# m-hamza-mughal/RAG-Gesture

Measured on AMD Instinct MI355X. Metric: SMPL-X frames/sec, len150 DDIM-50 + insertion guidance; 1/2/4/8 GPU, higher is better.
Workload: dtype bf16

## Files before the change

include/rg_gesture.h:

```cpp
#ifndef RG_GESTURE_H
#define RG_GESTURE_H

#include <stdint.h>

#ifdef __cplusplus
extern "C" {
#endif

typedef struct rg_handle rg_handle;

enum rg_status {
  RG_OK = 0,
  RG_ERR_INVALID = -1,
  RG_ERR_HIP = -2,
  RG_ERR_NO_DEVICE = -3
};

#define RG_VERSION 123
int rg_version(void);
int rg_create(rg_handle** out, int device);
void rg_destroy(rg_handle* h);
const char* rg_last_error(rg_handle* h);
int rg_num_cus(rg_handle* h);

int rg_ddim_update(rg_handle* h, const float* x, const float* x0, float* x_out, int64_t n,
                   float c_recip, float c_recipm1, float c_a, float c_b, void* stream);

int rg_cfg_ddim_update(rg_handle* h, const float* out, const float* x, float* x_out, float* x0_out,
                       const float* js, int B, int T, int D, float w_c, float w_u,
                       float c_recip, float c_recipm1, float c_a, float c_b, void* stream);
int rg_cfg_ddim_update_rows(rg_handle* h, const float* out_cond, const float* out_uncond, const float* x, float* x_out,
                            float* x_out2, const float* js, int B, int T, int D, float w_c, float w_u,
                            float c_recip, float c_recipm1, float c_a, float c_b, void* stream);

int rg_cfg_ddpm_update(rg_handle* h, const float* out, const float* x, const float* noise, float* x_out,
                       const float* js, int B, int T, int D, float w_c, float w_u, float c1, float c2, float sigma,
                       void* stream);

typedef struct rg_glue_args {
  const float* out_c_a;
  const float* out_u_a;
// ... 156 lines not shown
  const void* ustream;
  const void* afrag;
  const float* x;
  const float* tbias;
  const float* src_mask;
  const float* qmask;
  float* head;
  float* dump;
  float* xbuf;
  void* gbuf;
  const int* form;
  int L, B, T, S;
  int step, step_b, split;
  int dump_stage, dump_layer;
  int pairs;
  int twin;
  int* glue_ctr;
  rg_glue_args glue;
} rg_seq_args;

int rg_seq_forward(rg_handle* h, const rg_seq_args* args_host, void* stream);
int rg_seq2_forward(rg_handle* h, const rg_seq_args* args_host, void* stream);

#define RG_LANE_STRIDE 32
int rg_seqx_forward(rg_handle* h, const rg_seq_args* args_host, void* stream);
int rg_lane_form(rg_handle* h, int* state, int lane, int nlanes, int narrow_wgs, int wide_wgs, int budget, void* stream);

typedef struct rg_venc_args {
  const void* wstream;
  const void* pstream;
  const float* x;
  float* out;
  float* xbuf;
  float* dump;
  int nseq, S, nb, dump_block;
  const int* post_rows;
  float* post_mu;
  float* post_logvar;
  int post_nrows, pad_;
} rg_venc_args;

int rg_venc_forward(rg_handle* h, const rg_venc_args* args_host, void* stream);
int rg_venc_forward_grouped(rg_handle* h, const rg_venc_args* args_host, int n, void* stream);

typedef struct rg_vdec_args {
  const void* wstream;
// ... 429 lines not shown
```

rag-gesture_amd/csrc/rg_seq.hip:

```cpp
#ifndef RG_SEQ_BODY_ONLY
#define RG_PACK2_ONE
#endif
#include "rg_common.h"
#include "rg_stationary.h"
#include "rg_tail.h"
#include "rg_seq_host.h"

namespace {

constexpr int RD = 7;
constexpr int UPL = RG_SEQ_UPL;
constexpr int OFF_P0 = 0;
constexpr int OFF_P1 = TP * 1024;
constexpr int OFF_RING = 2 * TP * 1024;
constexpr int MAX_SEG = 8 * 34 + 5;
constexpr int OFF_DESC = OFF_RING + NW * RD * 1024;
constexpr int OFF_STAT = OFF_DESC + MAX_SEG * 16;
constexpr int LDS_BYTES = OFF_STAT + NW * TP * 2 * 4;
static_assert(LDS_BYTES <= 160 * 1024, "LDS budget");

#define U(name) U_##name = RG_SEQ_U_##name
enum { U(KV), U(KV2), U(Q), U(SAO), U(MIXX), U(Q3_0), U(MIX_0), U(Q3_1), U(MIX_1), U(Q3_2), U(MIX_2), U(FF1_0), U(FF2_0), U(FF1_1), U(FF2_1), U(FFO) };
#undef U
#define SEG(u, k) ((u) << 2 | (k))
// ... 460 lines not shown
  Acc out;
  zero(out);
  unit(out, P0, TL);
#pragma unroll
  for (int tb = 0; tb < 3; ++tb) {
    const int t = 16 * tb + l15;
    if (t < T) {
#pragma unroll
      for (int j = 0; j < 4; ++j) {
        const size_t o = ((size_t)seq * T + t) * DM + 64 * wave + 16 * j + 4 * g4;
        rg_tail::store_head(a.head, (unsigned)(o * 4), out[j][tb]);
      }
    }
  }
  wait_vmcnt<0>();
#ifdef RG_STAMPS
  if (a.dump_stage == 99 && lane0 == 0) {
    tacc[5] = __builtin_amdgcn_s_memrealtime() - tk0;
    for (int i = 0; i < 6; ++i) a.dump[(seq * 8 + wave) * 8 + i] = (float)tacc[i];
  }
#endif
}

__device__ __forceinline__ void seq_block(const rg_seq_args& a, const int block, const int pairs, unsigned char* const smem) {
  const int B = a.B;
  int seq0 = block;
  if (!pairs && (B & 3) == 0) {
    const int x = block & 7, q = block >> 3;
    seq0 = x < 4 ? 4 * q + x : B + 4 * q + (x - 4);
  }
  const int npass = pairs ? 2 : 1;
#pragma unroll 1
  for (int pass = 0; pass < npass; ++pass) {
    run_sequence(a, seq0 + pass * B, smem);
    __syncthreads();
    int* const ctr = rg_tail::late_ctr();
    if (ctr && !a.dump_stage) {
      const int c = seq0 + pass * B - (seq0 + pass * B >= B ? B : 0);
      rg_tail::arrive_and_glue<NTH>(ctr, c, c, reinterpret_cast<int*>(smem), __builtin_amdgcn_readfirstlane(threadIdx.x >> 6));
    }
  }
}

#ifndef RG_SEQ_BODY_ONLY
__global__ void __launch_bounds__(NTH) rg_seq_kernel(const rg_seq_args a) {
  extern __shared__ __attribute__((aligned(16))) unsigned char smem[];
  RG_OWN_THE_SIMD();
  seq_block(a, blockIdx.x, a.pairs, smem);
}

extern "C" int rg_seq_forward(rg_handle* h, const rg_seq_args* args_host, void* stream) {
  const std::string why = rg_seq_refusal(RG_SEQ_ENTRY, args_host);
  if (!why.empty()) { if (h) h->err = why; return RG_ERR_INVALID; }
  const rg_seq_args& a = *args_host;
  static rg_attr_once lds_once;
  RG_RESERVE_LDS(h, lds_once, rg_seq_kernel, LDS_BYTES);
  rg_prof_scope prof(h, stream, 3, rg_seq_flops(a));
  hipLaunchKernelGGL(rg_seq_kernel, dim3(a.pairs ? a.B : 2 * a.B), dim3(NTH), LDS_BYTES, rg_stream(stream), a);
  RG_CHECK_LAUNCH(h);
  prof.stop();
  return RG_OK;
}
#endif
```

rag-gesture_amd/csrc/rg_seq_host.h:

```cpp
#pragma once
#include <string>

#include "../../include/rg_gesture.h"

struct rg_seq_entry { const char *name, *need_bufs, *need_form, *no_dump, *twin_range, *twin_pairs, *no_twin; };
constexpr rg_seq_entry RG_SEQ_ENTRY = {"rg_seq_forward", nullptr, nullptr, nullptr, nullptr, nullptr, nullptr};
constexpr rg_seq_entry RG_SEQ2_ENTRY = {"rg_seq2_forward", "the two-sequence forward needs its scratch buffers xbuf and gbuf", nullptr,
                                        nullptr, "twin must be 0 or 1", "twin and pairs are two launch forms: set one of them", nullptr};
constexpr rg_seq_entry RG_SEQX_ENTRY = {
    "rg_seqx_forward", "the two-sequence form needs its scratch buffers xbuf and gbuf", "form: the lane's flag (rg_lane_form) must be given",
    "diagnostic dumps: use rg_seq_forward / rg_seq2_forward", nullptr, nullptr,
    "the twin form (one clip per workgroup) is not one of the device-chosen forms: use rg_seq2_forward"};

inline bool rg_seq_glue_ok(const rg_seq_args& a) {
  if (!a.glue_ctr) return true;
  const rg_glue_args& g = a.glue;
  if (a.dump_stage || g.n_a < 0 || g.n_b < 0 || g.n_a + g.n_b != a.B || g.T != a.T || g.D != 512 || !g.js || g.g_iter_next < 0) return false;
  if (g.n_a && !(g.out_c_a && g.out_u_a && g.x_a)) return false;
  if (g.n_b && !(g.out_c_b && g.out_u_b && g.x_b)) return false;
  return !g.in_seq_next || g.noise_next;
}

inline std::string rg_seq_refusal(const rg_seq_entry& e, const rg_seq_args* args) {
  const char* why = nullptr;
  if (!args) {
    why = "null args";
  } else {
    const rg_seq_args& a = *args;
    if (!(a.wstream && a.pstream && a.ustream && a.afrag && a.x && a.tbias && a.src_mask && a.qmask && a.head)) why = "null pointer";
    else if (e.need_bufs && !(a.xbuf && a.gbuf)) why = e.need_bufs;
    else if (e.need_form && !a.form) why = e.need_form;
    else if (!(a.L >= 1 && a.L <= 8 && a.B >= 1 && a.T >= 1 && a.T <= 48)) why = "unsupported shape (T <= 48, L <= 8)";
    else if (!(a.step >= 0 && a.step < a.S && a.step_b >= 0 && a.step_b < a.S)) why = "step out of range";
    else if (e.no_dump && a.dump_stage != 0) why = e.no_dump;
    else if (!e.no_dump && a.dump_stage != 0 && !a.dump) why = "dump_stage needs a dump buffer";
    else if (!(a.pairs == 0 || a.pairs == 1)) why = "pairs must be 0 or 1";
    else if (e.twin_range && !(a.twin == 0 || a.twin == 1)) why = e.twin_range;
    else if (e.twin_pairs && a.twin && a.pairs) why = e.twin_pairs;
    else if (e.no_twin && a.twin) why = e.no_twin;
    else if (!rg_seq_glue_ok(a)) why = "glue_ctr: glue must cover the B clips (n_a + n_b == B, T, D = 512), its pointers set, no dump";
  }
  return why ? std::string(e.name) + ": " + why : std::string();
}

inline double rg_seq_flops(const rg_seq_args& a) {
  const double unit = 2.0 * a.T * 512 * 512, att = 2.0 * a.T * 32 * 32 * 16;
  const double cond = (RG_SEQ_UPL * a.L + 2) * unit + a.L * (2 + 3) * att, unc = (10 * a.L + 2) * unit + a.L * 2 * att;
  return a.B * (cond + unc);
}
```

rag-gesture_amd/csrc/rg_tail.h:

```cpp
#pragma once
#include "rg_common.h"
#include <cstddef>

namespace rg_tail {

typedef __attribute__((ext_vector_type(4))) float f32x4;
typedef __attribute__((ext_vector_type(4))) unsigned u32x4;
constexpr int COHERENT = 17;

__device__ __forceinline__ float ddim_one(float x, float x0, float c_recip, float c_recipm1, float c_a, float c_b) {
#pragma clang fp contract(off)
  float eps = (c_recip * x - x0) / c_recipm1;
  return x0 * c_a + c_b * eps;
}
__device__ __forceinline__ float cfg_one(float oc, float ou, float jc, float ju, float w_c, float w_u) {
#pragma clang fp contract(off)
  return oc * w_c * jc + ou * w_u * ju;
}

template <typename P>
__device__ __forceinline__ P* uniform_ptr(P* p) {
  const unsigned long long v = reinterpret_cast<unsigned long long>(p);
  return reinterpret_cast<P*>((unsigned long long)__builtin_amdgcn_readfirstlane((unsigned)(v >> 32)) << 32 |
                              (unsigned)__builtin_amdgcn_readfirstlane((unsigned)v));
// ... 119 lines not shown
          const float4 v = glue_elem(a, k, C[i][h], U[i][h], X[i][h], jc[i], ju, ins, Y[i][h], E[i][h], two_over_numel);
          gstore(x0 + o, lane + 64 * h, v);
          if (x2_0) gstore(x2_0 + o, lane + 64 * h, v);
        }
      }
    }
  }
}

__device__ __forceinline__ float two_over_numel(const rg_glue_args& a) {
#pragma clang fp contract(off)
  const int rows_a = a.n_a * a.T;
  return 2.0f / ((float)rows_a * (float)a.D);
}

template <typename T>
__device__ __forceinline__ T late_arg(const unsigned offset) {
  auto p = (const __attribute__((address_space(4))) char*)__builtin_amdgcn_kernarg_segment_ptr();
  asm volatile("" : "+s"(p));
  T v;
  __builtin_memcpy(&v, p + offset, sizeof(T));
  return v;
}
__device__ __forceinline__ int* late_ctr() { return late_arg<int*>(offsetof(rg_seq_args, glue_ctr)); }

__device__ __forceinline__ void store_head(float* head, const unsigned byte_offset, const f32x4 v) {
  const auto rs = __builtin_amdgcn_make_buffer_rsrc(head, 0, 0x7fffffff, 0x00020000);
  __builtin_amdgcn_raw_buffer_store_b128(__builtin_bit_cast(u32x4, v), rs, byte_offset, 0, COHERENT);
}

template <int NTH>
__device__ __forceinline__ void arrive_and_glue(int* const ctr, const int c0, const int c1, int* const flag, const int wave) {
  const int lane = __builtin_amdgcn_mbcnt_hi(~0u, __builtin_amdgcn_mbcnt_lo(~0u, 0u));
  if (wave == 0 && lane == 0) {
    int m = 0;
    if (__hip_atomic_fetch_add(ctr + c0, 1, __ATOMIC_RELAXED, __HIP_MEMORY_SCOPE_AGENT) & 1) m |= 1;
    if (c1 != c0 && (__hip_atomic_fetch_add(ctr + c1, 1, __ATOMIC_RELAXED, __HIP_MEMORY_SCOPE_AGENT) & 1)) m |= 2;
    *flag = m;
  }
  __syncthreads();
  const int m = *flag;
  __syncthreads();
  if (m == 0) return;
  const rg_glue_args g = late_arg<rg_glue_args>(offsetof(rg_seq_args, glue));
  const float ton = two_over_numel(g);
#pragma unroll 1
  for (int q = 0; q < 2; ++q) {
    if (!(m >> q & 1)) continue;
    const int c = q ? c1 : c0;
    const bool ga = c < g.n_a;
    const int cl = ga ? c : c - g.n_a;
    glue_clip<NTH / 64>(g, ga, cl, wave, lane, ton);
  }
}

template <int NTH>
__device__ __forceinline__ void glue_own(const int c, const int wave) {
  const int lane = __builtin_amdgcn_mbcnt_hi(~0u, __builtin_amdgcn_mbcnt_lo(~0u, 0u));
  const rg_glue_args g = late_arg<rg_glue_args>(offsetof(rg_seq_args, glue));
  const bool ga = c < g.n_a;
  glue_clip<NTH / 64>(g, ga, ga ? c : c - g.n_a, wave, lane, two_over_numel(g));
}
}
```

rag-gesture_amd/denoiser.py:

```python
import math

import numpy as np
import torch

from . import capi, gemm as G, seqfwd as SQ

CONDS = ("xf_text", "xf_audio", "xf_spk")
BLOCKS = ("sa_block", "ca_blocks.xf_text", "ca_blocks.xf_audio", "ca_blocks.xf_spk", "ffn")


def _timestep_embedding(timesteps, dim, max_period=10000):
    half = dim // 2
    freqs = torch.exp(-math.log(max_period) * torch.arange(0, half, dtype=torch.float32) / half)
    args = timesteps[:, None].float() * freqs[None]
    return torch.cat([torch.cos(args), torch.sin(args)], dim=-1)


class DenoiserWeights:

    KV_GROUP = 2

    @staticmethod
    def _fold_ln(W, b, gamma, beta, pw, f32):
        Wp = (W.double() * gamma.double()[None, :]).float()
# ... 319 lines not shown
            pool[key] = torch.empty(*shape, device=self.w.dev, dtype=dtype)
        return pool[key]

    def chain_end(self):
        if self.sq is not None:
            self.sq.chain_end()

    def forward(self, x, step, step_b=None, split=None, glue=None):
        w, h, B, R, M, D, T = self.w, self.h, self.B, self.R, self.M, self.w.D, self.w.T
        if split is not None and not (0 < split < B):
            step, step_b, split = (step if split >= B else step_b), None, None
        if self.sq is not None:
            if glue is not None and not x.is_contiguous():
                raise capi.RgError("DenoiserSession.forward(glue=...): x is updated in place and must be contiguous")
            return self.sq.run(x.contiguous(), step, step_b, split, glue=glue)
        if glue is not None:
            raise capi.RgError("DenoiserSession.forward(glue=...): the sequence-stationary engine only")
        if self.ln_mode == "auto":
            out = self._forward_guarded(x, step)
            if split is None:
                return out
        return self._forward_chain(x, step, step_b, split)

    LN_GUARD_SIGMAS = 3.0

    def _forward_guarded(self, x, step):
        if torch.cuda.is_current_stream_capturing():
            raise capi.RgError("DenoiserSession(ln_mode='auto'): run one forward before capturing a graph")
        self._guard = torch.zeros(1, device=self.w.dev)
        self.ln_mode = "folded"
        out = self._forward_chain(x, step)
        self.ln_ratio = float(self._guard.item())
        self._guard = None
        if self.ln_ratio > self.LN_GUARD_SIGMAS ** 2:
            self.ln_mode, self.xa_bf = "prologue", None
            out = self._forward_chain(x, step)
        return out

    def _guard_stats(self, stats):
        if getattr(self, "_guard", None) is not None:
            self.h.call("ln_guard", stats, self.M, stats.shape[1], self.w.D, self._guard)

    def _forward_chain(self, x, step, step_b=None, split=None):
        w, h, B, R, M, D, T = self.w, self.h, self.B, self.R, self.M, self.w.D, self.w.T
        two = split is not None
        if two and (self.abf is None or self.hcat is None):
# ... 114 lines not shown
```

rag-gesture_amd/pipeline.py:

```python
import collections
import ctypes
import contextlib
import copy
import os
import time
import types

import torch
import yaml

from . import capi, denoiser, sampler, schedule as sched_mod, seqfwd, vae as vae_mod

MODELS = {}


def register_module(cls):
    MODELS[cls.__name__] = cls
    return cls


def register_with_mmcv(force=False):
    regs = []
    try:
        from mmcv.cnn import MODELS as mmcv_models
# ... 253 lines not shown
        self._ready()
        return {k: copy.deepcopy(v, memo) for k, v in dict.items(self) if k not in self._PLAIN}

    def __reduce__(self):
        self._ready()
        return (dict, (), None, None, iter([(k, v) for k, v in dict.items(self) if k not in self._PLAIN]))


@register_module
class MotionDiffusion(torch.nn.Module):

    profile_phases = False
    rotation_lanes = None
    form_lanes = None
    _cur_rot = None
    _last_state = None

    def __init__(self, model=None, loss_recon=None, loss_gen=None, loss_contact=None, loss_laplace=None,
                 diffusion_train=None, diffusion_test=None, init_cfg=None, inference_type="ddpm",
                 genloss_acceleration_weight=True, genloss_hands_weight=2, genloss_smooth=True,
                 body_part_lossweights=None, device="cuda", precision="bf16", lanes=2, sample_lanes=None, session_options=None,
                 vae_options=None, async_results=False, slots=2, max_inflight=2, cobatch_lanes="batch", base_lanes=8,
                 batch_lanes=4, lane_streams=None, calibrate_lanes=True, decode_stream=False, dynamic_forms=False, dynamic_budget=None, invert_alone_wide=True, tail_glue=True,
                 cache_exemplar_latents=True, exemplar_cache_bytes=8 << 30, skip_clip_encode=True, grouped_decode=True, **kwargs):
        super().__init__()
        self.grouped_decode = bool(grouped_decode)
        self.cache_exemplar_latents, self.exemplar_cache_bytes = bool(cache_exemplar_latents), int(exemplar_cache_bytes)
        self.skip_clip_encode = bool(skip_clip_encode)
        self.model = build_submodule(model, device=device, **kwargs)
        dt = dict(diffusion_test)
        self.schedule = sched_mod.Schedule(beta_scheduler=dt["beta_scheduler"], diffusion_steps=dt["diffusion_steps"],
                                           respace=dt.get("respace"))
        capi.require(dt.get("model_mean_type", "start_x") == "start_x" and dt.get("classifier_free_guidance_scale", 0) == 0,
                "unsupported argument: requires dt.get(\"model_mean_type\", \"start_x\") == \"start_x\" and dt.get(\"classifier_free_guidance_scale\", 0) == 0")
        self.inference_type = inference_type
        capi.require(inference_type in ("ddim", "ddpm"), "inference_type is 'ddim' (shipped config) or 'ddpm'")
        self.device, self.precision = torch.device(device), precision
        self.training = False
        self.session_options, self.vae_options = dict(session_options or {}), dict(vae_options or {})
        self.vae_options.setdefault("grouped_decode", self.grouped_decode)
        self._state = None
        self._sessions = {}
        self._graphs = {}
        self.use_graphs = True
        self.graph_captures = self.graph_cross_stream_waits = 0
        self._jitter = None
        self.phase_ms = {}
        self.lanes = int(lanes)
# ... 61 lines not shown

    def state_dict(self, *args, destination=None, prefix="", keep_vars=False):
        out = collections.OrderedDict() if destination is None else destination
        for k, v in (self._state or {}).items():
            out[prefix + "model." + k] = v
        return out

    _RECORD = True

    @staticmethod
    def _used_on(stream, *tensors):
        if not MotionDiffusion._RECORD:
            return
        for t in tensors:
            if torch.is_tensor(t) and t.is_cuda:
                t.record_stream(stream)

    def _graph_run(self, key, inputs, fn, owner=None):
        cur = torch.cuda.current_stream()
        self._used_on(cur, *inputs.values())
        if not self.use_graphs:
            return fn(inputs)
        if owner is not None:
            key = key + self._form_tag(self._session_opts(owner[0], owner[1], owner[2]))
        ent = self._graphs.pop(key, None)
        if ent is not None:
            self._graphs[key] = ent
        if ent is None:
            torch.cuda.synchronize()
            while len(self._graphs) >= self.MAX_GRAPHS:
                old = next(iter(self._graphs))
                del self._graphs[old]
                self._graph_owner.pop(old, None)
            if owner is not None:
                self._graph_owner[key] = owner
            static = {k: (None if v is None else torch.empty(v.shape, dtype=v.dtype, device=v.device).copy_(v))
                      for k, v in inputs.items()}
            side = torch.cuda.Stream()
            side.wait_stream(cur)
            with torch.cuda.stream(side):
                fn(static)
            cur.wait_stream(side)
            for k, v in inputs.items():
                if v is not None:
                    static[k].copy_(v)
            graph = torch.cuda.CUDAGraph()
            with capi.capture(graph):
# ... 39 lines not shown
        yield
        torch.cuda.synchronize()
        self.phase_ms[name] = self.phase_ms.get(name, 0.0) + (time.perf_counter() - t0) * 1e3

    def cuda(self, *a, **k):
        return self

    def cpu(self):
        return self

    def to(self, *a, **k):
        return self

    MAX_SESSIONS, MAX_GRAPHS = 192, 768

    def _session(self, B, role="sample", lane=0):
        opts = self._session_opts(B, role, lane)
        key = (B, role, lane, self._slot) + self._form_tag(opts)
        if key not in self._sessions:
            while len(self._sessions) >= self.MAX_SESSIONS:
                old = next(iter(self._sessions))
                torch.cuda.synchronize()
                del self._sessions[old]
                for gk in [g for g, o in self._graph_owner.items() if o == old[:4]]:
                    self._graphs.pop(gk, None)
                    del self._graph_owner[gk]
            self._sessions[key] = denoiser.DenoiserSession(self.model.weights, B, **opts)
        else:
            self._sessions[key] = self._sessions.pop(key)
        return self._sessions[key]

    LANE_SLOTS = 32

    @staticmethod
    def _form_tag(opts):
        return (bool(opts.get("seq_pairs")), opts.get("seq_duo"), "lane_dyn" in opts, bool(opts.get("seq_twin")))

    def _session_opts(self, B, role, lane):
        opts = dict(self.session_options)
        opts.setdefault("tail_glue", self.tail_glue)
        may_twin, twin = bool(opts.get("seq_twin", True)), False
        if opts.get("seq_pairs", "auto") == "auto":
            opts["seq_pairs"], duo = self._seq_form_auto(B)
            twin = may_twin and not opts["seq_pairs"] and bool(duo) and opts.get("seq_duo") is None
            if opts.get("seq_duo") is None:
                opts["seq_duo"] = duo
            if opts["seq_pairs"] and opts["seq_duo"] and role == "invert":
# ... 253 lines not shown
            prev_latent = prev_latent.to(dev).float()
            masked = torch.zeros_like(prev_latent)
            for idx in (up_i, ha_i, fa_i, lt_i):
                h.call("copy_rows", prev_latent, masked, B, 1, D, T, idx[-1], T, idx[0])
            prev_latent = masked

        ddpm = self.inference_type == "ddpm"
        in_seq = None
        if use_prev_latent and prev_latent is not None and not ddpm:
            in_seq = prev_latent
        elif use_outpaint and not ddpm:
            in_seq = retrieval_motion_latents
        x, start_noise, invl, inseq_noise, ddpm_noise = draw_batch_noise(
            tape, dev, B, T, D, S, use_inversion, use_insertion_guidance, visualize_inversion, ddpm, in_seq is not None,
            [len(retrieval_dict["retr_uncropped_latents"][b]) for b in range(B)] if use_inversion and visualize_inversion else ())
        st = types.SimpleNamespace(
            B=B, T=T, D=D, S=S, n_lat=n_lat, plan=plan, plan_s=plan_s, main=main, run_async=run_async, results=results,
            retrieval_dict=retrieval_dict, x=x, start_noise=start_noise, invl=invl, in_seq=in_seq, inseq_noise=inseq_noise,
            ddpm=ddpm, ddpm_noise=ddpm_noise, x_out=torch.empty(B, T, D, device=dev), use_inversion=use_inversion,
            use_insertion_guidance=use_insertion_guidance, guidance_iters=guidance_iters, guidance_lr=guidance_lr,
            visualize_inversion=visualize_inversion, inversion_start_time=inversion_start_time, vis_inv=[], vis_pairs=[],
            word=word, audio=audio, spk=spk, motion_mask=motion_mask, qmask=qmask, early_cond=early_cond,
            use_prev_latent=use_prev_latent, prev_latent=prev_latent, idx_groups=(up_i, ha_i, fa_i, lt_i), slot=self._slot, pid=pid, seq=self._submitted, via_submit=cob is not None,
            prev_future=prev_future if in_seq is not None else None, latent_ready=None)
        st.handle = self._last_state = types.SimpleNamespace(B=B, x_out=st.x_out, latent_ready=None)
        if cob is not None:
            st.word, st.audio, st.spk = (t.to(dev).clone() for t in (word, audio, spk))
            return self._submit_chain(st)
        self._inversion_pass(st)
        self._sampling_pass(st)
        return self._tail(st)

    def pending_latent(self):
        if self._last_state is None:
            raise capi.RgError("pending_latent(): no batch has been submitted")
        return PendingLatent(self._last_state)

    def _fill_prev(self, st, stream):
        pf = st.prev_future
        if pf is None:
            return
        st.prev_future = None
        src = pf.state
        if src.latent_ready is None:
            raise capi.RgError("prev_latent: the batch this pending latent belongs to has not been queued for sampling yet "
                               "(submit the windows in order)")
        stream.wait_event(src.latent_ready)
        self._used_on(stream, src.x_out, st.in_seq)
        with torch.cuda.stream(stream):
            lat = self.model.post_process(src.x_out)
            if pf.rows is not None:
                lat = lat.index_select(0, torch.tensor(pf.rows, device="cpu").pin_memory().to(self.device, non_blocking=True))
            h = self.model.weights.h
            for idx in st.idx_groups:
                h.call("copy_rows", lat.contiguous(), st.in_seq, st.B, 1, st.D, st.T, idx[-1], st.T, idx[0])

    def _take_slot(self, pid, main, lanes):
        slot = self._slots[pid] = (self._slots.get(pid, 0) + 1) % self.slots
        self._wait_slot(main, lanes, slot)
        self._slot = slot
        return slot

    def _wait_slot(self, main, lanes, slot):
        for lane in dict.fromkeys(lanes):
            for ev in self._slot_done.get((lane, slot), ()):
                main.wait_event(ev)

    @staticmethod
    def _lanes_of(*plans):
        return list(dict.fromkeys(lane for plan in plans for lane, _, _, _ in plan))

    def submit(self, **kwargs):
        if not self.async_results or self.slots < 2:
            raise capi.RgError("submit() needs MotionDiffusion(async_results=True, slots >= 2)")
        self._cob = dict(lane=self._submitted if (self.cobatch_lanes == "batch" and self.batch_lanes > 1) else None)
        self._submitted += 1
        try:
            self.forward(**kwargs)
        finally:
            self._cob = None
        return self._ready.popleft() if self._ready else None

    def flush(self):
        cob, self._cob = self._cob, dict(lane=0)
        try:
            self._finish_pending()
        finally:
            self._cob = cob
        out = list(self._ready)
        self._ready.clear()
        return out

    def _finish_alone(self, st):
        main = st.main = torch.cuda.current_stream()
        st.slot = self._take_slot(st.pid, main, self._lanes_of(st.plan_s))
        for lane, stream, b0, b1 in st.plan_s:
            self._sample_conditions(lane, b0, b1, st.word, st.audio, st.spk, st.motion_mask, st.qmask)
        self._sampling_pass(st)
        return self._tail(st)

    def _pending_upto(self, seq):
        return sorted((p for p in self._pend if self._pend[p].seq <= seq), key=lambda p: self._pend[p].seq)

    def _finish_pending(self, upto=None, resume=None):
        for p in self._pending_upto(float("inf") if upto is None else upto):
            self._ready.append(self._finish_alone(self._pend.pop(p)))
        if resume is not None:
            self._slot = self._slots[resume.pid] = resume.slot

    def _set_conditions_pair(self, sess, key, own, a, b, n_a):
        dev = self.model.weights.dev
        ins = {}
        for tag, (word, audio, spk, mask, qm) in (("a", a), ("b", b)):
            ins["word_" + tag], ins["audio_" + tag] = word.to(dev).float(), audio.to(dev).float()
            ins["spk_" + tag], ins["mask_" + tag] = spk.to(dev).long(), mask.to(dev).float()
            for c in denoiser.CONDS:
                ins["q_%s_%s" % (c, tag)] = qm[c].to(dev).float()

        def run(st):
            for tag, off, fin in (("a", 0, False), ("b", n_a, True)):
                sess.set_conditions(st["word_" + tag], st["audio_" + tag], st["spk_" + tag], st["mask_" + tag],
                                    {c: st["q_%s_%s" % (c, tag)] for c in denoiser.CONDS}, offset=off, finalize=fin)
            return ()
        self._graph_run(key + tuple(tuple(v.shape) for v in ins.values()), ins, run, owner=own)

    def _submit_chain(self, st):
        pend, S, T, D, dev = self._pend.get(st.pid), st.S, st.T, st.D, self.device
        lanes = [(lane, stream, b0, b1, self._exemplars(st, b0, b1)) for lane, stream, b0, b1 in st.plan] if st.use_inversion else []
        so = self.session_options
        groups_ok = self.precision == "bf16" and (self._runs_seq_engine(so) or so.get("styl_prepass", True))
        can_defer = (groups_ok and st.use_inversion and not st.visualize_inversion and not st.ddpm and st.plan == st.plan_s
# ... 152 lines not shown
                    elif st.use_insertion_guidance:
                        gi, lr = tuple(int(v) for v in st.guidance_iters), float(st.guidance_lr)
                        key = ("guided", Bl, lane, T, self._slot, in_seq is not None, gi, lr)
                        (xl,) = self._graph_run(key, loop_in, lambda s, sess=sess, gi=gi, lr=lr: (
                            sampler.ddim_guided_sample_loop(sess, s["x"], s["invl"], gi, lr, s["noise"], in_seq=s["in_seq"]),),
                            owner=okey)
                    else:
                        key = ("sample", Bl, lane, T, self._slot, in_seq is not None)
                        (xl,) = self._graph_run(key, loop_in, lambda s, sess=sess: (sampler.ddim_sample_loop(
                            sess, s["x"], in_seq=s["in_seq"], inseq_noise=s["noise"]),), owner=okey)
                    st.x_out[b0:b1].copy_(xl)

    def _tail(self, st):
        gre, results, main, S, T, D, B = self.model.gesture_rep_encoder, st.results, st.main, st.S, st.T, st.D, st.B
        tail_lane, tail = st.plan_s[self._tail_turn % len(st.plan_s)][:2] if st.run_async else (-1, main)
        if st.run_async and self.decode_on_own_stream and self._decode_stream is not None:
            tail_lane, tail = -2, self._decode_stream
        self._tail_turn += 1
        if st.run_async and st.via_submit:
            capi.require(st.seq >= self._last_out_seq, "internal: results handed out against the submission order")
            self._last_out_seq = st.seq
        if self._jitter is not None:
            self._jitter(tail, "tail")
        for _, stream, _, _ in st.plan + st.plan_s:
            if stream is not tail:
                tail.wait_stream(stream)
        st.latent_ready = st.handle.latent_ready = tail.record_event()
        self._used_on(tail, st.x_out, *st.vis_inv, *st.vis_pairs)
        with torch.cuda.stream(tail):
            output = self.model.post_process(st.x_out)
            results["prev_latentout"] = output
            with self._phase("vae_decode"):
                up, lo, fa, ha, tr, ex_, co = self._graph_run(("dec", B, gre.part_streams is None, tail_lane), dict(z=output),
                                                                lambda s: gre.decode(s["z"]))
            results["pred_upper"], results["pred_lower"], results["pred_facepose"] = up, lo, fa
            results["pred_hands"], results["pred_transl"], results["pred_exps"] = ha, tr, ex_
            results["pred_contact"] = co
            if st.use_inversion and st.visualize_inversion and st.vis_inv:
                n_ex = len(st.vis_inv)
                keys = ("upper", "lower", "facepose", "hands", "transl", "exps")
                for name, lat, k in (("inverted_output", torch.stack(st.vis_inv).reshape(n_ex * S, T, D), S),
                                     ("reconspair_output", torch.stack(st.vis_pairs).reshape(n_ex * 2, T, D), 2)):
                    lat = self.model.post_process(lat.contiguous())
                    parts = [[] for _ in keys]
                    for c0 in range(0, lat.shape[0], 128):
                        dec = gre.decode(lat[c0:c0 + 128].contiguous())
                        for j in range(6):
# ... 20 lines not shown
```

rag-gesture_amd/sampler.py:

```python
import ctypes

import torch

from . import capi

from .seqfwd import GlueArgs

SPLICE_MAX = capi.header_constants()["RG_SPLICE_MAX"]
SpliceTable = capi.struct("rg_splice_table")


TAIL_GLUE = True


def _tail_ok(sess, x):
    return (TAIL_GLUE and getattr(sess, "tail_glue", True) and getattr(sess, "sq", None) is not None and sess.h.recorder is None and x.is_cuda and x.is_contiguous()
            and x.dtype == torch.float32 and x.shape[0] == sess.B)


def _p(t):
    if t is None:
        return None
    if not (t.is_cuda and t.is_contiguous() and t.dtype == torch.float32):
        raise capi.RgError("rg_cobatch_glue: contiguous fp32 device tensors expected")
    return t.data_ptr()


def _glue(sess, lr=0.0, *, i=None, x_a=None, n_a=0, nxt=None, noise_nxt=None, g_next=0, k=None, x_b=None, keep_b=None, n_b=0):
    sch, w, head, B, T = sess.w.schedule, sess.w, sess.head, sess.B, sess.w.T
# ... 34 lines not shown
    x_all, k, x_b, keep_b = inv
    sess.forward(x_all, i, step_b=k, split=n)
    sess.cfg_ddim_rows(0, n, x, x, i, sch.c_prev_a[i], sch.c_prev_b[i])
    sess.cfg_ddim_rows(n, sess.B - n, x_b, x_b, k, sch.c_next_a[k], sch.c_next_b[k], x_out2=keep_b)


def _sample_loop(sess, x, in_seq, inseq_noise, inverted=None, guidance_iters=None, lr=0.0):
    S = sess.w.schedule.num_timesteps
    if _tail_ok(sess, x):
        _insert_first(sess, x, sess.B, in_seq, inseq_noise)
        for i in range(S - 1, -1, -1):
            nxt = None if i == 0 else (inverted[i - 1] if inverted is not None else in_seq)
            sess.forward(x, i, glue=_glue(sess, lr, i=i, x_a=x, n_a=sess.B, nxt=nxt, noise_nxt=None if nxt is None else inseq_noise[i - 1],
                                          g_next=guidance_iters[i - 1] if inverted is not None and i > 0 else 0))
        sess.chain_end()
        return x
    for i in range(S - 1, -1, -1):
        g_iter = None
        if inverted is not None and i != S - 1:
            in_seq, g_iter = inverted[i], guidance_iters[i]
        _step(sess, x, i, in_seq, None if in_seq is None else inseq_noise[i], g_iter, lr)
    sess.chain_end()
    return x


def ddim_sample_loop(sess, x, in_seq=None, inseq_noise=None):
    return _sample_loop(sess, x, in_seq, inseq_noise)


def p_sample_loop(sess, x, noise):
    S = sess.w.schedule.num_timesteps
    for i in range(S - 1, -1, -1):
        sess.forward(x, i)
        sess.cfg_ddpm(x, x, i, noise[i])
    sess.chain_end()
    return x


def ddim_reverse_sample_loop(sess, x, out):
    sch = sess.w.schedule
    if _tail_ok(sess, x) and out.is_contiguous() and out.dtype == torch.float32:
        for i in range(sch.num_timesteps):
            sess.forward(x, i, glue=_glue(sess, k=i, x_b=x, keep_b=out[i], n_b=sess.B))
        sess.chain_end()
        return out
    cur = x
# ... 62 lines not shown
```

rag-gesture_amd/seqfwd.py:

```python
import ctypes

import torch

from . import capi

_C = capi.header_constants()
UPL = _C["RG_SEQ_UPL"]
(U_KV, U_KV2, U_Q, U_SAO, U_MIXX, U_Q3_0, U_MIX_0, U_Q3_1, U_MIX_1, U_Q3_2, U_MIX_2, U_FF1_0, U_FF2_0, U_FF1_1, U_FF2_1, U_FFO) = (
    _C["RG_SEQ_U_" + n] for n in "KV KV2 Q SAO MIXX Q3_0 MIX_0 Q3_1 MIX_1 Q3_2 MIX_2 FF1_0 FF2_0 FF1_1 FF2_1 FFO".split())
CONDS = ("xf_text", "xf_audio", "xf_spk")
LANE_STRIDE = _C["RG_LANE_STRIDE"]
GlueArgs = capi.struct("rg_glue_args")
SeqArgs = capi.struct("rg_seq_args")


def supported(cfg, T, precision):
    return (precision == "bf16" and cfg["latent_dim"] == 512 and cfg["num_heads"] == 16 and cfg["ff_size"] == 1024
            and T <= 48 and 1 <= cfg["num_layers"] <= 8)


def pack_unit(W):
    capi.require(W.shape == (512, 512), "unsupported argument: requires W.shape == (512, 512)")
    v = W.to(torch.bfloat16).view(8, 4, 16, 16, 4, 8)
    return v.permute(0, 3, 1, 4, 2, 5).contiguous().view(8, 64, 64, 8)
# ... 108 lines not shown
        a.wstream, a.pstream, a.ustream, a.afrag = p(self.st.wstream), p(self.st.pstream), p(self.st.ustream), p(self.afrag)
        a.tbias, a.src_mask, a.qmask, a.head = p(w.tbias), p(sess.src_mask), p(sess.qmask), p(sess.head)
        a.L, a.B, a.T, a.S = w.L, B, w.T, self.st.S
        a.pairs = int(bool(pairs))
        a.twin = int(self.twin)
        a.dump, a.dump_stage, a.dump_layer = None, 0, 0
        a.xbuf = p(self.xbuf) if self.xbuf is not None else None
        a.gbuf = p(self.gbuf) if self.gbuf is not None else None
        self._entry = "seq2_forward" if self.duo else "seq_forward"
        self.lane_dyn = None
        if lane_dyn is not None:
            state, lane, n, budget = lane_dyn
            if not (state.is_cuda and state.dtype == torch.int32 and state.is_contiguous() and state.numel() >= LANE_STRIDE * n and 0 <= lane < n):
                raise capi.RgError("lane_dyn: state must be a contiguous device int32 tensor [n, %d], 0 <= lane < n" % LANE_STRIDE)
            self.lane_dyn = (state, int(lane), int(n), int(budget))
            a.form = state.data_ptr() + 4 * (LANE_STRIDE * lane + 1)
            if self.duo:
                self._entry = "seqx_forward"
        self._fn = getattr(self.h.lib, "rg_" + self._entry)

    def set_a(self, a_pre, o0, o1):
        self.afrag[:, :, o0:o1] = a_fragments(a_pre)

    def run(self, x, step, step_b=None, split=None, dump=None, dump_stage=0, dump_layer=0, glue=None):
        a = self.args
        if glue is not None:
            if glue.n_a + glue.n_b != self.sess.B or glue.T != self.sess.w.T or glue.D != self.sess.w.D or dump_stage:
                raise capi.RgError("rg_seq_forward: the tail's groups must cover the session's clips (n_a + n_b == B)")
            a.glue, a.glue_ctr = glue, self.glue_ctr.data_ptr()
        else:
            a.glue_ctr = None
        if not (x.is_contiguous() and x.dtype == torch.float32 and x.numel() == self.sess.B * self.sess.w.T * self.sess.w.D):
            raise capi.RgError("rg_seq_forward: x must be a contiguous fp32 [B, T, D] tensor")
        a.x, a.step = x.data_ptr(), int(step)
        a.step_b = int(step if step_b is None else step_b)
        a.split = int(self.sess.B if split is None else split)
        a.dump = dump.data_ptr() if dump is not None else None
        a.dump_stage, a.dump_layer = int(dump_stage), int(dump_layer)
        if self.lane_dyn is not None and not dump_stage:
            state, lane, n, budget = self.lane_dyn
            B = self.sess.B
            wide = 2 * B
            if self.duo:
                sp = max(0, min(B, a.split))
                npc = (sp + 1) // 2 + (B - sp + 1) // 2
                narrow = npc if a.pairs else 2 * npc
            else:
                narrow = wide = B if a.pairs else 2 * B
            self.h.call("lane_form", state, lane, n, narrow, wide, budget)
        self.h.call("seq2_forward" if dump_stage and self.lane_dyn is not None and self.duo else self._entry, ctypes.byref(a))
        return self.sess.head

    def chain_end(self):
        if self.lane_dyn is not None:
            state, lane, n, budget = self.lane_dyn
            self.h.call("lane_form", state, lane, n, 0, 0, budget)
```

Measured before the change: 67530.

## Drain pending lane requests through one grouped sequence-forward launch per step

Adds rg_seq_forward_many, which packs up to eight sessions' argument blocks into one kernarg block and launches one grid covering all their sequences. Each workgroup picks its session from the cumulative block ends, and the tail-glue late-argument reads are offset accordingly. On the Python side, pending requests that each sit alone on a lane with compatible settings are drained together: one stream runs a grouped DDIM loop, captured as a graph, instead of separate per-lane loops. This is meant to fill the GPU better and cut launch count when several small requests are in flight, at the cost of cross-stream waits and a larger kernarg block.

```diff
diff --git a/include/rg_gesture.h b/include/rg_gesture.h
--- a/include/rg_gesture.h
+++ b/include/rg_gesture.h
@@ -16,7 +16,7 @@
   RG_ERR_NO_DEVICE = -3
 };
 
-#define RG_VERSION 123
+#define RG_VERSION 124
 int rg_version(void);
 int rg_create(rg_handle** out, int device);
 void rg_destroy(rg_handle* h);
@@ -219,6 +219,9 @@
 int rg_seq_forward(rg_handle* h, const rg_seq_args* args_host, void* stream);
 int rg_seq2_forward(rg_handle* h, const rg_seq_args* args_host, void* stream);
 
+#define RG_SEQ_MANY_MAX 8
+int rg_seq_forward_many(rg_handle* h, const rg_seq_args* const* args_host, int n, void* stream);
+
 #define RG_LANE_STRIDE 32
 int rg_seqx_forward(rg_handle* h, const rg_seq_args* args_host, void* stream);
 int rg_lane_form(rg_handle* h, int* state, int lane, int nlanes, int narrow_wgs, int wide_wgs, int budget, void* stream);
diff --git a/rag-gesture_amd/csrc/rg_seq.hip b/rag-gesture_amd/csrc/rg_seq.hip
--- a/rag-gesture_amd/csrc/rg_seq.hip
+++ b/rag-gesture_amd/csrc/rg_seq.hip
@@ -506,7 +506,8 @@
 #endif
 }
 
-__device__ __forceinline__ void seq_block(const rg_seq_args& a, const int block, const int pairs, unsigned char* const smem) {
+__device__ __forceinline__ void seq_block(const rg_seq_args& a, const int block, const int pairs, unsigned char* const smem,
+                                          const unsigned arg_base = 0) {
   const int B = a.B;
   int seq0 = block;
   if (!pairs && (B & 3) == 0) {
@@ -518,10 +519,10 @@
   for (int pass = 0; pass < npass; ++pass) {
     run_sequence(a, seq0 + pass * B, smem);
     __syncthreads();
-    int* const ctr = rg_tail::late_ctr();
+    int* const ctr = rg_tail::late_ctr(arg_base);
     if (ctr && !a.dump_stage) {
       const int c = seq0 + pass * B - (seq0 + pass * B >= B ? B : 0);
-      rg_tail::arrive_and_glue<NTH>(ctr, c, c, reinterpret_cast<int*>(smem), __builtin_amdgcn_readfirstlane(threadIdx.x >> 6));
+      rg_tail::arrive_and_glue<NTH>(ctr, c, c, reinterpret_cast<int*>(smem), __builtin_amdgcn_readfirstlane(threadIdx.x >> 6), arg_base);
     }
   }
 }
@@ -545,4 +546,45 @@
   prof.stop();
   return RG_OK;
 }
+
+struct rg_seq_many_block {
+  rg_seq_args a[RG_SEQ_MANY_MAX];
+  int end[RG_SEQ_MANY_MAX];
+};
+static_assert(sizeof(rg_seq_many_block) <= 4096, "the parameter block must fit the kernarg segment");
+
+__global__ void __launch_bounds__(NTH) rg_seq_many_kernel(const rg_seq_many_block p) {
+  extern __shared__ __attribute__((aligned(16))) unsigned char smem[];
+  RG_OWN_THE_SIMD();
+  const int block = blockIdx.x;
+  int s = 0, first = 0;
+#pragma unroll
+  for (int i = 0; i + 1 < RG_SEQ_MANY_MAX; ++i)
+    if (block >= p.end[i]) { s = i + 1; first = p.end[i]; }
+  s = __builtin_amdgcn_readfirstlane(s);
+  seq_block(p.a[s], block - first, 0, smem, (unsigned)(offsetof(rg_seq_many_block, a) + s * sizeof(rg_seq_args)));
+}
+
+extern "C" int rg_seq_forward_many(rg_handle* h, const rg_seq_args* const* args_host, int n, void* stream) {
+  const std::string why = rg_seq_many_refusal(args_host, n);
+  if (!why.empty()) { if (h) h->err = why; return RG_ERR_INVALID; }
+  rg_seq_many_block p{};
+  int total = 0;
+  double flops = 0.0;
+  for (int i = 0; i < RG_SEQ_MANY_MAX; ++i) {
+    if (i < n) {
+      p.a[i] = *args_host[i];
+      total += 2 * p.a[i].B;
+      flops += rg_seq_flops(p.a[i]);
+    }
+    p.end[i] = total;
+  }
+  static rg_attr_once lds_once;
+  RG_RESERVE_LDS(h, lds_once, rg_seq_many_kernel, LDS_BYTES);
+  rg_prof_scope prof(h, stream, 3, flops);
+  hipLaunchKernelGGL(rg_seq_many_kernel, dim3(total), dim3(NTH), LDS_BYTES, rg_stream(stream), p);
+  RG_CHECK_LAUNCH(h);
+  prof.stop();
+  return RG_OK;
+}
 #endif
diff --git a/rag-gesture_amd/csrc/rg_seq_host.h b/rag-gesture_amd/csrc/rg_seq_host.h
--- a/rag-gesture_amd/csrc/rg_seq_host.h
+++ b/rag-gesture_amd/csrc/rg_seq_host.h
@@ -43,6 +43,25 @@
   return why ? std::string(e.name) + ": " + why : std::string();
 }
 
+constexpr rg_seq_entry RG_SEQ_MANY_ENTRY = {"rg_seq_forward_many", nullptr, nullptr, "diagnostic dumps: use rg_seq_forward", nullptr, nullptr,
+                                            "the twin form is rg_seq2_forward's: a grouped launch runs one workgroup per sequence"};
+
+inline std::string rg_seq_many_refusal(const rg_seq_args* const* args, const int n) {
+  const std::string name = std::string(RG_SEQ_MANY_ENTRY.name) + ": ";
+  if (!args || n < 1) return name + "null or empty list of sessions";
+  if (n > RG_SEQ_MANY_MAX) return name + "too many sessions (at most RG_SEQ_MANY_MAX)";
+  for (int i = 0; i < n; ++i) {
+    const std::string why = rg_seq_refusal(RG_SEQ_MANY_ENTRY, args[i]);
+    if (!why.empty()) return why;
+    const rg_seq_args &a = *args[i], &a0 = *args[0];
+    if (a.pairs) return name + "pairs is another launch form: a grouped launch runs one workgroup per sequence";
+    if (!(a.L == a0.L && a.T == a0.T && a.S == a0.S)) return name + "the sessions must agree in L, T and S";
+    if (!(a.wstream == a0.wstream && a.pstream == a0.pstream && a.ustream == a0.ustream))
+      return name + "the sessions must share the weight, parameter and table streams";
+  }
+  return std::string();
+}
+
 inline double rg_seq_flops(const rg_seq_args& a) {
   const double unit = 2.0 * a.T * 512 * 512, att = 2.0 * a.T * 32 * 32 * 16;
   const double cond = (RG_SEQ_UPL * a.L + 2) * unit + a.L * (2 + 3) * att, unc = (10 * a.L + 2) * unit + a.L * 2 * att;
diff --git a/rag-gesture_amd/csrc/rg_tail.h b/rag-gesture_amd/csrc/rg_tail.h
--- a/rag-gesture_amd/csrc/rg_tail.h
+++ b/rag-gesture_amd/csrc/rg_tail.h
@@ -165,7 +165,7 @@
   __builtin_memcpy(&v, p + offset, sizeof(T));
   return v;
 }
-__device__ __forceinline__ int* late_ctr() { return late_arg<int*>(offsetof(rg_seq_args, glue_ctr)); }
+__device__ __forceinline__ int* late_ctr(const unsigned base = 0) { return late_arg<int*>(base + offsetof(rg_seq_args, glue_ctr)); }
 
 __device__ __forceinline__ void store_head(float* head, const unsigned byte_offset, const f32x4 v) {
   const auto rs = __builtin_amdgcn_make_buffer_rsrc(head, 0, 0x7fffffff, 0x00020000);
@@ -173,7 +173,8 @@
 }
 
 template <int NTH>
-__device__ __forceinline__ void arrive_and_glue(int* const ctr, const int c0, const int c1, int* const flag, const int wave) {
+__device__ __forceinline__ void arrive_and_glue(int* const ctr, const int c0, const int c1, int* const flag, const int wave,
+                                                const unsigned base = 0) {
   const int lane = __builtin_amdgcn_mbcnt_hi(~0u, __builtin_amdgcn_mbcnt_lo(~0u, 0u));
   if (wave == 0 && lane == 0) {
     int m = 0;
@@ -185,7 +186,7 @@
   const int m = *flag;
   __syncthreads();
   if (m == 0) return;
-  const rg_glue_args g = late_arg<rg_glue_args>(offsetof(rg_seq_args, glue));
+  const rg_glue_args g = late_arg<rg_glue_args>(base + offsetof(rg_seq_args, glue));
   const float ton = two_over_numel(g);
 #pragma unroll 1
   for (int q = 0; q < 2; ++q) {
diff --git a/rag-gesture_amd/denoiser.py b/rag-gesture_amd/denoiser.py
--- a/rag-gesture_amd/denoiser.py
+++ b/rag-gesture_amd/denoiser.py
@@ -365,6 +365,13 @@
                 return out
         return self._forward_chain(x, step, step_b, split)
 
+    @staticmethod
+    def forward_many(sessions, calls):
+        for s, kw in zip(sessions, calls):
+            if s.sq is None or not kw["x"].is_contiguous():
+                raise capi.RgError("DenoiserSession.forward_many: the sequence-stationary engine only, x contiguous")
+        return SQ.run_many([s.sq for s in sessions], calls)
+
     LN_GUARD_SIGMAS = 3.0
 
     def _forward_guarded(self, x, step):
diff --git a/rag-gesture_amd/pipeline.py b/rag-gesture_amd/pipeline.py
--- a/rag-gesture_amd/pipeline.py
+++ b/rag-gesture_amd/pipeline.py
@@ -299,8 +299,10 @@
                  body_part_lossweights=None, device="cuda", precision="bf16", lanes=2, sample_lanes=None, session_options=None,
                  vae_options=None, async_results=False, slots=2, max_inflight=2, cobatch_lanes="batch", base_lanes=8,
                  batch_lanes=4, lane_streams=None, calibrate_lanes=True, decode_stream=False, dynamic_forms=False, dynamic_budget=None, invert_alone_wide=True, tail_glue=True,
-                 cache_exemplar_latents=True, exemplar_cache_bytes=8 << 30, skip_clip_encode=True, grouped_decode=True, **kwargs):
+                 cache_exemplar_latents=True, exemplar_cache_bytes=8 << 30, skip_clip_encode=True, grouped_decode=True,
+                 grouped_drain=True, **kwargs):
         super().__init__()
+        self.grouped_drain = bool(grouped_drain)
         self.grouped_decode = bool(grouped_decode)
         self.cache_exemplar_latents, self.exemplar_cache_bytes = bool(cache_exemplar_latents), int(exemplar_cache_bytes)
         self.skip_clip_encode = bool(skip_clip_encode)
@@ -408,7 +410,8 @@
         if not self.use_graphs:
             return fn(inputs)
         if owner is not None:
-            key = key + self._form_tag(self._session_opts(owner[0], owner[1], owner[2]))
+            for o in (owner if isinstance(owner[0], tuple) else (owner,)):
+                key = key + self._form_tag(self._session_opts(o[0], o[1], o[2]))
         ent = self._graphs.pop(key, None)
         if ent is not None:
             self._graphs[key] = ent
@@ -494,7 +497,7 @@
                 old = next(iter(self._sessions))
                 torch.cuda.synchronize()
                 del self._sessions[old]
-                for gk in [g for g, o in self._graph_owner.items() if o == old[:4]]:
+                for gk in [g for g, o in self._graph_owner.items() if o == old[:4] or old[:4] in o]:
                     self._graphs.pop(gk, None)
                     del self._graph_owner[gk]
             self._sessions[key] = denoiser.DenoiserSession(self.model.weights, B, **opts)
@@ -794,7 +797,7 @@
             visualize_inversion=visualize_inversion, inversion_start_time=inversion_start_time, vis_inv=[], vis_pairs=[],
             word=word, audio=audio, spk=spk, motion_mask=motion_mask, qmask=qmask, early_cond=early_cond,
             use_prev_latent=use_prev_latent, prev_latent=prev_latent, idx_groups=(up_i, ha_i, fa_i, lt_i), slot=self._slot, pid=pid, seq=self._submitted, via_submit=cob is not None,
-            prev_future=prev_future if in_seq is not None else None, latent_ready=None)
+            prev_future=prev_future if in_seq is not None else None, latent_ready=None, wait_streams=())
         st.handle = self._last_state = types.SimpleNamespace(B=B, x_out=st.x_out, latent_ready=None)
         if cob is not None:
             st.word, st.audio, st.spk = (t.to(dev).clone() for t in (word, audio, spk))
@@ -827,8 +830,8 @@
             for idx in st.idx_groups:
                 h.call("copy_rows", lat.contiguous(), st.in_seq, st.B, 1, st.D, st.T, idx[-1], st.T, idx[0])
 
-    def _take_slot(self, pid, main, lanes):
-        slot = self._slots[pid] = (self._slots.get(pid, 0) + 1) % self.slots
+    def _take_slot(self, pid, main, lanes, slot=None):
+        slot = self._slots[pid] = (self._slots.get(pid, 0) + 1) % self.slots if slot is None else slot
         self._wait_slot(main, lanes, slot)
         self._slot = slot
         return slot
@@ -875,10 +878,72 @@
         return sorted((p for p in self._pend if self._pend[p].seq <= seq), key=lambda p: self._pend[p].seq)
 
     def _finish_pending(self, upto=None, resume=None):
-        for p in self._pending_upto(float("inf") if upto is None else upto):
-            self._ready.append(self._finish_alone(self._pend.pop(p)))
+        sts = [self._pend.pop(p) for p in self._pending_upto(float("inf") if upto is None else upto)]
+        group = self._drain_group(sts) if self.grouped_drain else []
+        if group:
+            self._drain_grouped(group)
+        for st in sts:
+            self._ready.append(self._tail(st) if any(st is g for g in group) else self._finish_alone(st))
         if resume is not None:
             self._slot = self._slots[resume.pid] = resume.slot
+
+    DRAIN_SLOT = 0
+
+    def _drain_group(self, sts):
+        sett = lambda st: (st.T, st.S, bool(st.use_insertion_guidance), tuple(int(v) for v in st.guidance_iters), float(st.guidance_lr))
+
+        def alone_on_a_lane(st):
+            return (st.run_async and st.via_submit and not st.ddpm and st.prev_future is None and st.plan == st.plan_s
+                    and len(st.plan_s) == 1 and tuple(st.plan_s[0][2:]) == (0, st.B))
+
+        def one_sequence_form(st):
+            o = self._session_opts(st.B, "sample", st.plan_s[0][0])
+            return (self._runs_seq_engine(o) and not o.get("seq_pairs") and not o.get("seq_duo") and not o["seq_twin"] and "lane_dyn" not in o
+                    and o["tail_glue"] and sampler.TAIL_GLUE and self.model.weights.h.recorder is None)
+        if self.precision != "bf16":
+            return []
+        group, lanes = [], set()
+        for st in sts:
+            if (len(group) < sampler.MANY_MAX and alone_on_a_lane(st) and st.plan_s[0][0] not in lanes and one_sequence_form(st)
+                    and (not group or sett(st) == sett(group[0]))):
+                group.append(st)
+                lanes.add(st.plan_s[0][0])
+        return group if len(group) >= 2 else []
+
+    def _drain_grouped(self, sts):
+        main = torch.cuda.current_stream()
+        sess = {}
+        for st in sts:
+            lane, _, b0, b1 = st.plan_s[0]
+            st.main = main
+            st.slot = self._take_slot(st.pid, main, [lane], slot=self.DRAIN_SLOT % self.slots)
+            self._sample_conditions(lane, b0, b1, st.word, st.audio, st.spk, st.motion_mask, st.qmask)
+            sess[id(st)] = self._session(st.B, "sample", lane)
+        order = sorted(sts, key=lambda st: st.plan_s[0][0])
+        n, g = len(order), order[0].plan_s[0][1]
+        g.wait_stream(main)
+        for st in order:
+            if st.plan_s[0][1] is not g:
+                g.wait_stream(st.plan_s[0][1])
+            self._used_on(g, st.x, st.in_seq, st.inseq_noise, st.invl, st.x_out)
+            st.wait_streams = [g]
+        guided = bool(order[0].use_insertion_guidance)
+        gi, lr = tuple(int(v) for v in order[0].guidance_iters), float(order[0].guidance_lr)
+        sessions = [sess[id(st)] for st in order]
+        ins = {}
+        for k, st in enumerate(order):
+            ins.update({"x%d" % k: st.x, "in_seq%d" % k: st.in_seq, "noise%d" % k: st.inseq_noise, "invl%d" % k: st.invl if guided else None})
+
+        def loop(s):
+            col = lambda name: [s["%s%d" % (name, k)] for k in range(n)]
+            return tuple(sampler.sample_loop_many(sessions, col("x"), col("in_seq"), col("noise"), col("invl") if guided else None,
+                                                  gi if guided else None, lr))
+        owners = tuple((st.B, "sample", st.plan_s[0][0], st.slot) for st in order)
+        key = ("guided_many" if guided else "sample_many", owners, order[0].T, tuple(st.in_seq is not None for st in order), gi, lr)
+        with torch.cuda.stream(g), self._phase("sampling"):
+            outs = self._graph_run(key, ins, loop, owner=owners)
+            for st, xl in zip(order, outs):
+                st.x_out.copy_(xl)
 
     def _set_conditions_pair(self, sess, key, own, a, b, n_a):
         dev = self.model.weights.dev
@@ -1077,7 +1142,7 @@
             self._last_out_seq = st.seq
         if self._jitter is not None:
             self._jitter(tail, "tail")
-        for _, stream, _, _ in st.plan + st.plan_s:
+        for stream in [s for _, s, _, _ in st.plan + st.plan_s] + list(st.wait_streams):
             if stream is not tail:
                 tail.wait_stream(stream)
         st.latent_ready = st.handle.latent_ready = tail.record_event()
diff --git a/rag-gesture_amd/sampler.py b/rag-gesture_amd/sampler.py
--- a/rag-gesture_amd/sampler.py
+++ b/rag-gesture_amd/sampler.py
@@ -4,7 +4,7 @@
 
 from . import capi
 
-from .seqfwd import GlueArgs
+from .seqfwd import GlueArgs, MANY_MAX
 
 SPLICE_MAX = capi.header_constants()["RG_SPLICE_MAX"]
 SpliceTable = capi.struct("rg_splice_table")
@@ -85,6 +85,36 @@
         _step(sess, x, i, in_seq, None if in_seq is None else inseq_noise[i], g_iter, lr)
     sess.chain_end()
     return x
+
+
+def many_ok(sessions, xs):
+    return (1 < len(sessions) <= MANY_MAX and all(_tail_ok(s, x) and s.sq.groupable() for s, x in zip(sessions, xs))
+            and all(s.w is sessions[0].w for s in sessions) and len({id(s) for s in sessions}) == len(sessions))
+
+
+def sample_loop_many(sessions, xs, in_seqs, inseq_noises, inverteds=None, guidance_iters=None, lr=0.0):
+    n = len(sessions)
+    inverteds = [None] * n if inverteds is None else inverteds
+    capi.require(all(v is None or len(guidance_iters) == sessions[0].w.schedule.num_timesteps == v.shape[0] for v in inverteds),
+                 "unsupported argument: requires len(guidance_iters) == S == inverted.shape[0]")
+    if not many_ok(sessions, xs):
+        for k in range(n):
+            _sample_loop(sessions[k], xs[k], in_seqs[k], inseq_noises[k], inverteds[k], guidance_iters, lr)
+        return xs
+    S = sessions[0].w.schedule.num_timesteps
+    for k, sess in enumerate(sessions):
+        _insert_first(sess, xs[k], sess.B, in_seqs[k], inseq_noises[k])
+    for i in range(S - 1, -1, -1):
+        calls = []
+        for k, sess in enumerate(sessions):
+            nxt = None if i == 0 else (inverteds[k][i - 1] if inverteds[k] is not None else in_seqs[k])
+            calls.append(dict(x=xs[k], step=i, glue=_glue(
+                sess, lr, i=i, x_a=xs[k], n_a=sess.B, nxt=nxt, noise_nxt=None if nxt is None else inseq_noises[k][i - 1],
+                g_next=guidance_iters[i - 1] if inverteds[k] is not None and i > 0 else 0)))
+        type(sessions[0]).forward_many(sessions, calls)
+    for sess in sessions:
+        sess.chain_end()
+    return xs
 
 
 def ddim_sample_loop(sess, x, in_seq=None, inseq_noise=None):
diff --git a/rag-gesture_amd/seqfwd.py b/rag-gesture_amd/seqfwd.py
--- a/rag-gesture_amd/seqfwd.py
+++ b/rag-gesture_amd/seqfwd.py
@@ -154,7 +154,7 @@
     def set_a(self, a_pre, o0, o1):
         self.afrag[:, :, o0:o1] = a_fragments(a_pre)
 
-    def run(self, x, step, step_b=None, split=None, dump=None, dump_stage=0, dump_layer=0, glue=None):
+    def _set_args(self, x, step, step_b=None, split=None, dump=None, dump_stage=0, dump_layer=0, glue=None):
         a = self.args
         if glue is not None:
             if glue.n_a + glue.n_b != self.sess.B or glue.T != self.sess.w.T or glue.D != self.sess.w.D or dump_stage:
@@ -169,6 +169,10 @@
         a.split = int(self.sess.B if split is None else split)
         a.dump = dump.data_ptr() if dump is not None else None
         a.dump_stage, a.dump_layer = int(dump_stage), int(dump_layer)
+        return a
+
+    def run(self, x, step, step_b=None, split=None, dump=None, dump_stage=0, dump_layer=0, glue=None):
+        a = self._set_args(x, step, step_b, split, dump, dump_stage, dump_layer, glue)
         if self.lane_dyn is not None and not dump_stage:
             state, lane, n, budget = self.lane_dyn
             B = self.sess.B
@@ -183,7 +187,24 @@
         self.h.call("seq2_forward" if dump_stage and self.lane_dyn is not None and self.duo else self._entry, ctypes.byref(a))
         return self.sess.head
 
+    def groupable(self):
+        return not self.duo and not self.twin and not self.args.pairs and self.lane_dyn is None
+
     def chain_end(self):
         if self.lane_dyn is not None:
             state, lane, n, budget = self.lane_dyn
             self.h.call("lane_form", state, lane, n, 0, 0, budget)
+
+
+MANY_MAX = _C["RG_SEQ_MANY_MAX"]
+
+
+def run_many(sqs, calls):
+    if not (1 <= len(sqs) <= MANY_MAX and len(sqs) == len(calls)):
+        raise capi.RgError("rg_seq_forward_many: 1 to %d sessions, one set of arguments each" % MANY_MAX)
+    if not all(sq.groupable() for sq in sqs):
+        raise capi.RgError("rg_seq_forward_many: sessions in the one-workgroup-per-sequence form only (no duo, pairs, twin or lane_dyn)")
+    args = [sq._set_args(**kw) for sq, kw in zip(sqs, calls)]
+    ptrs = (ctypes.c_void_p * len(args))(*[ctypes.addressof(a) for a in args])
+    sqs[0].h.call("seq_forward_many", ctypes.cast(ptrs, ctypes.c_void_p), len(args))
+    return [sq.sess.head for sq in sqs]
```

Measured after the change: 70640, median of 6. +4.6%, better.
